# wanmeihuali/taichi_3d_gaussian_splatting

Hardware: NVIDIA H100
Metric: rendered Mpix/sec fwd+bwd @1080p, 1e6 Gaussians (higher is better)
Workload: dtype f32

## Files before the change

### taichi_3d_gaussian_splatting_b200/csrc/blend_bwd.cu

```cuda
#include "blend_bwd.cuh"

namespace gsb {

__device__ __forceinline__ void warp_transpose_reduce11(float (&v)[11], int lane) {
    {
        const bool hi = lane & 16;
#pragma unroll
        for (int i = 0; i < 5; ++i) {
            const float send = hi ? v[i] : v[i + 6];
            const float keep = hi ? v[i + 6] : v[i];
            v[i] = keep + __shfl_xor_sync(0xffffffffu, send, 16);
        }
        v[5] += __shfl_xor_sync(0xffffffffu, v[5], 16);
    }
    {
        const bool hi = lane & 8;
#pragma unroll
        for (int i = 0; i < 3; ++i) {
            const float send = hi ? v[i] : v[i + 3];
            const float keep = hi ? v[i + 3] : v[i];
            v[i] = keep + __shfl_xor_sync(0xffffffffu, send, 8);
        }
    }
    {
// ... 93 lines not shown
        if (block_start < warp_last) {
            const int skip = block_end - warp_last;
#pragma unroll 1
            for (int lw = skip > 0 ? (skip >> 5) : 0; lw < 8; ++lw) {
                unsigned int bits = s_bits[buf][warp][lw];
                if (skip > lw * 32) bits &= ~((1u << (skip - lw * 32)) - 1u);
                while (bits) {
                    const int j = lw * 32 + __ffs(bits) - 1;
                    bits &= bits - 1;
                    const int idx = block_end - 1 - j;
                    float v[11];
                    bool contributes;
                    {
                        const unsigned int ja = sb + j * 16;
                        const float4 r0 = lds128<0>(ja);
                        const float4 r1 = lds128<PLANE>(ja);
                        const float4 r2 = lds128<2 * PLANE>(ja);
                        const float d0 = px - r0.x, d1 = py - r0.y;
                        const float q0 = r0.z * d0 + r0.w * d1;
                        const float q1 = r0.w * d0 + r1.x * d1;
                        if (EXACT_EXP) {
                            const float gp = expf(-0.5f * (d0 * q0 + d1 * q1)) * r1.y;
                            const float opa = r1.z;
                            const float prod_alpha = gp * opa;
                            contributes = (idx < last) && (prod_alpha >= 1.0f / 255.0f);
                            const float alpha = fminf(prod_alpha, 0.99f);
                            const float inv = 1.0f / (1.0f - alpha);
                            const float Tn = T * inv;
                            const float aT = contributes ? alpha * Tn : 0.0f;
                            const float a_grad = contributes ? (r2.x * Tn - w0 * inv) * g0 + (r2.y * Tn - w1 * inv) * g1 +
                                                                   (r2.z * Tn - w2 * inv) * g2
                                                             : 0.0f;
                            T = contributes ? Tn : T;
                            w0 = fmaf(r2.x, aT, w0);
                            w1 = fmaf(r2.y, aT, w1);
                            w2 = fmaf(r2.z, aT, w2);
                            const float G = a_grad * opa * gp;
                            const float vs0 = G * q0, vs1 = G * q1;
                            if (STATS) {
                                mag0 += fabsf(vs0);
                                mag1 += fabsf(vs1);
                            }
                            v[0] = vs0;
                            v[1] = vs1;
                            v[2] = vs0 * q0;
                            v[3] = vs0 * q1;
                            v[4] = vs1 * q1;
                            v[5] = aT * g0;
                            v[6] = aT * g1;
                            v[7] = aT * g2;
                            v[8] = a_grad * gp * (1.0f - opa) * opa;
                            v[9] = STATS ? sqrtf(vs0 * vs0 + vs1 * vs1) : 0.0f;
                        } else {
                            const float P = fast_alpha(d0, d1, (-0.5f * GSB_L2E) * r0.z, -GSB_L2E * r0.w,
                                                       (-0.5f * GSB_L2E) * r1.x, r1.y);
                            contributes = (idx < last) && (P >= 1.0f / 255.0f);
                            const float alpha = fminf(P, 0.99f);
                            const float inv = rcp_approx(1.0f - alpha);
                            const float Tn = T * inv;
                            const float aT = contributes ? alpha * Tn : 0.0f;
                            const float cg = fmaf(r2.z, g2, fmaf(r2.y, g1, r2.x * g0));
                            const float a_grad = contributes ? fmaf(cg, Tn, -(w0 * inv)) : 0.0f;
                            T = contributes ? Tn : T;
                            w0 = fmaf(cg, aT, w0);
                            const float G = a_grad * P;
                            const float vs0 = G * q0, vs1 = G * q1;
                            if (STATS) {
                                mag0 += fabsf(vs0);
                                mag1 += fabsf(vs1);
                            }
                            v[0] = vs0;
                            v[1] = vs1;
                            v[2] = vs0 * q0;
                            v[3] = vs0 * q1;
                            v[4] = vs1 * q1;
                            v[5] = aT * g0;
                            v[6] = aT * g1;
                            v[7] = aT * g2;
                            v[8] = G * r1.z;
                            v[9] = STATS ? sqrt_approx(vs0 * vs0 + vs1 * vs1) : 0.0f;
                        }
                        v[10] = (STATS && contributes) ? 1.0f : 0.0f;
                    }
                    if (lane == 0) GSB_EMU_COUNT(EC_BF_VISITS, 1);
                    GSB_EMU_COUNT(EC_BF_PAIRS, contributes ? 1 : 0);
                    if (__any_sync(0xffffffffu, contributes)) {
                        if (lane == 0) GSB_EMU_COUNT(EC_BF_VISITS_ANY, 1);
                        warp_transpose_reduce11(v, lane);
                        if (red_writer && (STATS || red_slot < 9))
                            atomicAdd(p.accum + (size_t)s_off[buf][j] * GSB_ACCUM_FLOATS + red_slot, v[0]);
                    }
                }
            }
        }
    }
    if (STATS) {
        p.mag_image[2 * pix] = mag0;
        p.mag_image[2 * pix + 1] = mag1;
    }
}

#ifndef GSB_HOST_EMU
static BlendBwdParams make_blend_bwd_params(const GsbBackwardArgs &a, const Workspace &ws);

int launch_blend_backward_work(const GsbBackwardArgs &a, const Workspace &ws, unsigned long long *counters_dev,
                               cudaStream_t stream) {
    BlendBwdParams p = make_blend_bwd_params(a, ws);
    p.work_counters = counters_dev;
// ... 621 lines not shown
```

### taichi_3d_gaussian_splatting_b200/csrc/blend_bwd_transposed.cu

```cuda
#include <type_traits>

#include "blend_bwd.cuh"

namespace gsb {

#ifndef GSB_TB_CHUNK
#define GSB_TB_CHUNK 16
#endif
#ifndef GSB_TB_MIN_BLOCKS
#if GSB_TB_CHUNK == 8
#define GSB_TB_MIN_BLOCKS 4
#else
#define GSB_TB_MIN_BLOCKS 3
#endif
#endif
constexpr int TB_CHUNK = GSB_TB_CHUNK;
static_assert(TB_CHUNK == 8 || TB_CHUNK == 16, "a phase-2 lane takes whole rows of the 8 x 4 patch");
constexpr int TB_ROWS = TB_CHUNK / 8;
constexpr int TB_ROW = TB_CHUNK + 1;

struct TbWarp {
    float4 g[32];
    float4 chunk[3][TB_CHUNK];
    float2 x[32 * TB_ROW];
// ... 38 lines not shown

#ifndef GSB_TB_P1_UNROLL
#define GSB_TB_P1_UNROLL 4
#endif
constexpr int TB_P1_UNROLL = GSB_TB_P1_UNROLL;
static_assert(TB_CHUNK % TB_P1_UNROLL == 0, "a full chunk is a whole number of phase-1 groups");
__device__ __forceinline__ void red_add_f32x4(float *addr, const float4 v) {
#ifdef GSB_HOST_EMU
    atomicAdd(addr, v.x);
    atomicAdd(addr + 1, v.y);
    atomicAdd(addr + 2, v.z);
    atomicAdd(addr + 3, v.w);
#else
    atomicAdd(reinterpret_cast<float4 *>(addr), v);
#endif
}
__device__ __forceinline__ float keep_if_contributing(float P, int idx, int last) {
#ifdef GSB_HOST_EMU
    return ((idx < last) && (P >= 1.0f / 255.0f)) ? P : 0.0f;
#else
    float r;
    asm("{\n"
        ".reg .pred p, q;\n"
        "setp.lt.s32 q, %2, %3;\n"
        "setp.ge.and.f32 p, %1, 0f3B808081, q;\n"
        "selp.f32 %0, %1, 0f00000000, p;\n"
        "}\n"
        : "=f"(r)
        : "f"(P), "r"(idx), "r"(last));
    return r;
#endif
}

template <int CF>
using TbParams = typename std::conditional<CF == 0, BlendBwdParams, BlendBwdFeatParams>::type;

template <bool EXACT_EXP, bool STATS, bool COUNT = false, bool DEPTH = false, bool ALPHA = false, int CF = 0>
__global__ void __launch_bounds__(GSB_TILE_PIXELS, tb_min_blocks(CF))
blend_backward_transposed_kernel(const TbParams<CF> p) {
    static_assert(!(COUNT && (DEPTH || ALPHA || CF)), "the work-counter diagnostic runs the default arithmetic only");
    static_assert(CF % 4 == 0 && CF <= 16, "features: whole float4 groups");
    TbShared &S = *reinterpret_cast<TbShared *>(tb_dynamic_smem());
    constexpr int NV = STATS ? 11 : 9;
    constexpr int CFW = CF > 0 ? CF : 4;
    constexpr int P1U = CF >= 16 ? 2 : TB_P1_UNROLL;
    TbFeat<CFW> &SF = *reinterpret_cast<TbFeat<CFW> *>(tb_dynamic_smem() + sizeof(TbShared));

    const int tile = blockIdx.x;
    const int tu = tile % p.tiles_x, tv = tile / p.tiles_x;
    const int tid = threadIdx.x, lane = tid & 31, warp = tid >> 5;
    const int pu = tu * GSB_TILE_WIDTH + (warp & 1) * 8 + (lane & 7);
    const int pv = tv * GSB_TILE_HEIGHT + (warp >> 1) * 4 + (lane >> 3);
    const float px = (float)pu + 0.5f, py = (float)pv + 0.5f;
    const size_t pix = (size_t)pv * p.W + pu;
    const int start = p.tile_start[tile];

    const int last = p.last_effective[pix];
    float T = 1.0f - p.acc_alpha[pix];
    float w0 = 0.0f, w1 = 0.0f, w2 = 0.0f;
    const float g0 = p.grad_image[3 * pix], g1 = p.grad_image[3 * pix + 1], g2 = p.grad_image[3 * pix + 2];
    float mag0 = 0.0f, mag1 = 0.0f;
    unsigned int n_visits = 0, n_pairs = 0;
    float gd = 0.0f, hd = 0.0f, w3 = 0.0f;
    if (DEPTH) {
        const float Sa = p.acc_alpha[pix];
        gd = Sa > 0.0f ? p.grad_depth[pix] / Sa : 0.0f;
        hd = EXACT_EXP ? p.depth[pix] : gd * p.depth[pix];
    }
    float ga = 0.0f;
    if (ALPHA) {
        const float gs = p.grad_alpha[pix];
        ga = EXACT_EXP ? gs * T : DEPTH ? gs - hd : gs;
    }
    TbWarp &Wp = S.w[warp];
    Wp.g[lane] = make_float4(g0, g1, g2, gd);
    float gf[CFW];
    float wF;
    typename TbFeat<CFW>::Warp &WF = SF.w[warp];
    const BlendFeatureParams fp = feature_params(p);
    const int C = CF > 0 ? fp.channels : 0;
    if constexpr (CF > 0) {
        wF = 0.0f;
        const float *src = fp.grad_feature_map + pix * C;
#pragma unroll
        for (int c = 0; c < CF; ++c) gf[c] = c < C ? src[c] : 0.0f;
#pragma unroll
        for (int c = 0; c < CF; c += 4) WF.g[lane][c / 4] = make_float4(gf[c], gf[c + 1], gf[c + 2], gf[c + 3]);
    }

    const int ci = lane % TB_CHUNK, row0 = (lane / TB_CHUNK) * TB_ROWS;
    float2 *const x = Wp.x;
    float4 *const fin = reinterpret_cast<float4 *>(x);
    unsigned char *const list = Wp.list;

    int warp_last = last;
#pragma unroll
    for (int d = 16; d > 0; d >>= 1) warp_last = max(warp_last, __shfl_xor_sync(0xffffffffu, warp_last, d));
    if (tid == 0) {
        S.max_last = start;
        S.origin = make_float2((float)(tu * GSB_TILE_WIDTH), (float)(tv * GSB_TILE_HEIGHT));
    }
    __syncthreads();
    if (lane == 0) atomicMax(&S.max_last, warp_last);
    __syncthreads();
    const int end = min(p.tile_end[tile], S.max_last);

// ... 12 lines not shown
            {
                const int idx = block_end - 1 - tid;
                unsigned int mask = 0;
                if (idx >= block_start) {
                    const int o = __ldg(&p.sorted_vals[idx]);
                    const float4 *rec = p.records + 3 * (size_t)o;
                    const float4 r0 = __ldg(rec), r1 = __ldg(rec + 1);
                    if (EXACT_EXP) {
                        s_r0[tid] = r0;
                        s_r1[tid] = r1;
                    } else {
                        float4 f0, f1;
                        fast_planes(r0, r1, f0, f1);
                        s_r0[tid] = f0;
                        s_r1[tid] = f1;
                    }
                    float4 r2 = __ldg(rec + 2);
                    r2.w = __int_as_float(o);
                    s_r2[tid] = r2;
                    if constexpr (CF > 0) SF.row[buf][tid] = __ldg(&fp.point_id[o]);
                    mask = splat_patch_mask(r0.x, r0.y, r0.z, r0.w, r1.x, r1.y * r1.z, S.origin.x, S.origin.y);
                }
#pragma unroll
                for (int w = 0; w < 8; ++w) {
                    const unsigned int bits = __ballot_sync(0xffffffffu, (mask >> w) & 1u);
                    if (lane == 0) S.bits[buf][w][warp] = bits;
                }
            }
            __syncthreads();
            if (tid == 0) GSB_EMU_COUNT(EC_BATCHES, 1);
            if (block_start < warp_last) {
                const int skip = block_end - warp_last;
#pragma unroll
                for (int k = 0; k < 8; ++k) {
                    unsigned int bits = S.bits[buf][warp][k];
                    const int lo = skip - 32 * k;
                    if (lo >= 32) bits = 0u;
                    else if (lo > 0) bits &= ~((1u << lo) - 1u);
                    if ((bits >> lane) & 1u)
                        list[count + __popc(bits & ((1u << lane) - 1u))] = (unsigned char)(k * 32 + lane);
                    count += __popc(bits);
                }
                __syncwarp();
            }
        }

        int pos = 0;
#pragma unroll 1
        do {
            if (pos < count) {
                const int take = min(TB_CHUNK - have, count - pos);
                if (lane < take) {
                    const int j = list[pos + lane], slot = have + lane;
                    ck0[slot] = s_r0[j];
                    ck1[slot] = s_r1[j];
                    float4 r2 = s_r2[j];
                    ck_off[slot] = __float_as_int(r2.w);
                    r2.w = __int_as_float(block_end - 1 - j);
                    ck2[slot] = r2;
                    if constexpr (CF > 0) {
                        const int row = SF.row[buf][j];
                        WF.row[slot] = row;
                        const float *src = fp.features + (size_t)row * C;
#pragma unroll
                        for (int c = 0; c < CF; c += 4)
                            WF.f[slot][c / 4] = make_float4(c < C ? __ldg(src + c) : 0.0f, c + 1 < C ? __ldg(src + c + 1) : 0.0f,
                                                            c + 2 < C ? __ldg(src + c + 2) : 0.0f,
                                                            c + 3 < C ? __ldg(src + c + 3) : 0.0f);
                    }
                }
                have += take;
                pos += take;
                __syncwarp();
            }
            if (have == TB_CHUNK || (!real && have > 0)) {
                const int n = have;
                have = 0;
                if (COUNT) n_visits += (lane == 0) ? (unsigned int)n : 0u;
                if (lane == 0) {
                    GSB_EMU_COUNT(EC_TB_SPLATS, n);
                    GSB_EMU_COUNT(EC_TB_CHUNKS, 1);
                }
                const auto p1 = [&](const int i) -> float2 {
                    const float4 r0 = ck0[i];
                    const float4 r1 = ck1[i];
                    const float4 r2 = ck2[i];
                    const int idx = __float_as_int(r2.w);
                    const float d0 = px - r0.x, d1 = py - r0.y;
                    float sf = 0.0f;
                    if constexpr (CF > 0) {
#pragma unroll
                        for (int c = 0; c < CF; c += 4) {
                            const float4 f = WF.f[i][c / 4];
                            sf = fmaf(gf[c], f.x, sf);
                            sf = fmaf(gf[c + 1], f.y, sf);
                            sf = fmaf(gf[c + 2], f.z, sf);
                            sf = fmaf(gf[c + 3], f.w, sf);
                        }
                    }
                    float G, aT;
                    if (EXACT_EXP) {
                        const float q0 = r0.z * d0 + r0.w * d1;
                        const float q1 = r0.w * d0 + r1.x * d1;
                        const float gp = expf(-0.5f * (d0 * q0 + d1 * q1)) * r1.y;
                        const float prod_alpha = gp * r1.z;
                        const bool contributes = (idx < last) && (prod_alpha >= 1.0f / 255.0f);
                        const float alpha = fminf(prod_alpha, 0.99f);
                        const float inv = 1.0f / (1.0f - alpha);
                        const float Tn = T * inv;
                        aT = contributes ? alpha * Tn : 0.0f;
                        float a_grad = contributes ? (r2.x * Tn - w0 * inv) * g0 + (r2.y * Tn - w1 * inv) * g1 +
                                                         (r2.z * Tn - w2 * inv) * g2
                                                   : 0.0f;
                        if (DEPTH) {
                            const float e = r1.w - hd;
                            a_grad += contributes ? (e * Tn - w3 * inv) * gd : 0.0f;
                            w3 = fmaf(e, aT, w3);
                        }
                        if (ALPHA) a_grad += contributes ? ga * inv : 0.0f;
                        if constexpr (CF > 0) {
                            a_grad += contributes ? sf * Tn - wF * inv : 0.0f;
                            wF = fmaf(sf, aT, wF);
                        }
                        T = contributes ? Tn : T;
                        w0 = fmaf(r2.x, aT, w0);
                        w1 = fmaf(r2.y, aT, w1);
                        w2 = fmaf(r2.z, aT, w2);
                        G = a_grad * r1.z * gp;
                        if (STATS) {
                            mag0 += fabsf(G * q0);
                            mag1 += fabsf(G * q1);
                        }
                    } else {
                        float P = fast_alpha(d0, d1, r0.z, r0.w, r1.x, r1.y);
                        P = keep_if_contributing(P, idx, last);
                        const float alpha = fminf(P, 0.99f);
                        const float inv = rcp_approx(1.0f - alpha);
                        T *= inv;
                        aT = alpha * T;
                        float cg = fmaf(r2.z, g2, fmaf(r2.y, g1, ALPHA ? fmaf(r2.x, g0, ga) : r2.x * g0));
                        if (DEPTH) cg = ALPHA ? fmaf(gd, r1.w, cg) : fmaf(gd, r1.w, cg) - hd;
                        if constexpr (CF > 0) cg += sf;
                        const float a_grad = fmaf(cg, T, -(w0 * inv));
                        w0 = fmaf(cg, aT, w0);
                        G = a_grad * P;
                        if (STATS) {
                            const float q0 = (-2.0f / GSB_L2E) * fmaf(r0.z, d0, 0.5f * r0.w * d1);
                            const float q1 = (-2.0f / GSB_L2E) * fmaf(0.5f * r0.w, d0, r1.x * d1);
                            mag0 += fabsf(G * q0);
                            mag1 += fabsf(G * q1);
                        }
                    }
                    if (COUNT) n_pairs += aT > 0.0f ? 1u : 0u;
                    return make_float2(G, aT);
                };
                if (n == TB_CHUNK) {
#pragma unroll 1
                    for (int i0 = 0; i0 < TB_CHUNK; i0 += P1U) {
                        float2 ex[P1U];
#pragma unroll
                        for (int u = 0; u < P1U; ++u) ex[u] = p1(i0 + u);
#pragma unroll
                        for (int u = 0; u < P1U; ++u) x[lane * TB_ROW + i0 + u] = ex[u];
                    }
                } else {
#pragma unroll 1
                    for (int i = 0; i < n; ++i) x[lane * TB_ROW + i] = p1(i);
                }
                __syncwarp();

                const bool active = ci < n;
                float4 s0 = ck0[active ? ci : 0];
                float4 s1 = ck1[active ? ci : 0];
                if (!EXACT_EXP) {
                    s0.z *= -2.0f / GSB_L2E;
                    s0.w *= -1.0f / GSB_L2E;
                    s1.x *= -2.0f / GSB_L2E;
                }
                const float ca = s0.z, cb = s0.w, cc = s1.x;
                const float2 org = S.origin;
                const float pxc = org.x + (float)((warp & 1) * 8) + 4.0f;
                const float pyb = org.y + (float)((warp >> 1) * 4 + row0) + 0.5f;
                const float dxc = pxc - s0.x;
                float acc[12];
#pragma unroll
                for (int k = 0; k < 12; ++k) acc[k] = 0.0f;
                float af[CFW];
                if constexpr (CF > 0) {
#pragma unroll
                    for (int c = 0; c < CF; ++c) af[c] = 0.0f;
                }
                unsigned int nz = 0u;
#pragma unroll
                for (int row = 0; row < TB_ROWS; ++row) {
                    const float d1 = (pyb + (float)row) - s0.y;
                    const float q0r = fmaf(ca, dxc, cb * d1);
                    const float q1r = fmaf(cb, dxc, cc * d1);
                    float m0 = 0.0f, m1 = 0.0f, m2 = 0.0f;
#pragma unroll
                    for (int k = 0; k < 8; ++k) {
                        const float kc = (float)k - 3.5f;
                        const int pp = 8 * (row0 + row) + k;
                        const float2 ga = x[pp * TB_ROW + ci];
                        const float4 gp = Wp.g[pp];
                        m0 += ga.x;
                        m1 = fmaf(kc, ga.x, m1);
                        m2 = fmaf(kc * kc, ga.x, m2);
                        acc[5] = fmaf(ga.y, gp.x, acc[5]);
                        acc[6] = fmaf(ga.y, gp.y, acc[6]);
                        acc[7] = fmaf(ga.y, gp.z, acc[7]);
                        if (DEPTH) acc[11] = fmaf(ga.y, gp.w, acc[11]);
                        if (STATS) {
                            const float vs0 = ga.x * fmaf(ca, kc, q0r), vs1 = ga.x * fmaf(cb, kc, q1r);
                            const float mm = vs0 * vs0 + vs1 * vs1;
                            acc[9] += EXACT_EXP ? sqrtf(mm) : sqrt_approx(mm);
                            acc[10] += ga.y > 0.0f ? 1.0f : 0.0f;
                        }
                        nz |= __float_as_uint(ga.y);
                    }
                    const float t0 = fmaf(ca, m1, q0r * m0), t1 = fmaf(cb, m1, q1r * m0);
                    const float u0 = fmaf(ca, m2, q0r * m1), u1 = fmaf(cb, m2, q1r * m1);
                    acc[0] += t0;
                    acc[1] += t1;
                    acc[2] += fmaf(ca, u0, q0r * t0);
                    acc[3] += fmaf(cb, u0, q1r * t0);
                    acc[4] += fmaf(cb, u1, q1r * t1);
                    acc[8] += m0;
                }
                if constexpr (CF > 0) {
#pragma unroll 1
                    for (int row = 0; row < TB_ROWS; ++row) {
#pragma unroll 4
                        for (int k = 0; k < 8; ++k) {
                            const int pp = 8 * (row0 + row) + k;
                            const float aT = x[pp * TB_ROW + ci].y;
#pragma unroll
                            for (int c = 0; c < CF; c += 4) {
                                const float4 gc = WF.g[pp][c / 4];
                                af[c] = fmaf(aT, gc.x, af[c]);
                                af[c + 1] = fmaf(aT, gc.y, af[c + 1]);
                                af[c + 2] = fmaf(aT, gc.z, af[c + 2]);
                                af[c + 3] = fmaf(aT, gc.w, af[c + 3]);
                            }
                        }
                    }
                }
#pragma unroll
                for (int d = TB_CHUNK; d < 32; d *= 2) {
#pragma unroll
                    for (int k = 0; k < NV; ++k) acc[k] += __shfl_xor_sync(0xffffffffu, acc[k], d);
                    if (DEPTH) acc[11] += __shfl_xor_sync(0xffffffffu, acc[11], d);
                    if constexpr (CF > 0) {
#pragma unroll
                        for (int c = 0; c < CF; ++c) af[c] += __shfl_xor_sync(0xffffffffu, af[c], d);
                    }
                    nz |= __shfl_xor_sync(0xffffffffu, nz, d);
                }
                if constexpr (CF > 0) if (active && nz != 0u) {
                    constexpr int parts = 32 / TB_CHUNK;
                    const int h = lane / TB_CHUNK;
                    float *dst = fp.grad_features + (size_t)WF.row[ci] * C;
#pragma unroll
                    for (int c = 0; c < CF; c += 4) {
                        if ((c / 4) % parts != h || c >= C) continue;
                        if (C % 4 == 0) {
                            red_add_f32x4(dst + c, make_float4(af[c], af[c + 1], af[c + 2], af[c + 3]));
                        } else {
#pragma unroll
                            for (int k = 0; k < 4; ++k)
                                if (c + k < C) atomicAdd(dst + c + k, af[c + k]);
                        }
                    }
                }
                acc[8] *= EXACT_EXP ? (1.0f - s1.z) : s1.z;
                __syncwarp();
                if (lane < TB_CHUNK) {
                    if (!(active && nz != 0u)) ck_off[ci] = -1;
                    else GSB_EMU_COUNT(EC_TB_ROWS, 1);
                    fin[3 * ci] = make_float4(acc[0], acc[1], acc[2], acc[3]);
                    fin[3 * ci + 1] = make_float4(acc[4], acc[5], acc[6], acc[7]);
                    fin[3 * ci + 2] = make_float4(acc[8], STATS ? acc[9] : 0.0f, STATS ? acc[10] : 0.0f,
                                                  DEPTH ? acc[11] : 0.0f);
                }
                __syncwarp();
#pragma unroll
                for (int e0 = 0; e0 < 3 * TB_CHUNK; e0 += 32) {
                    const int e = e0 + lane, row = e / 3;
                    if (e < 3 * TB_CHUNK) {
                        const int o = ck_off[row];
                        if (o >= 0) red_add_f32x4(p.accum + (size_t)o * GSB_ACCUM_FLOATS + 4 * (e - 3 * row), fin[e]);
                    }
                }
                __syncwarp();
            }
        } while (pos < count);
        if (!real) break;
    }
    if (STATS) {
        p.mag_image[2 * pix] = mag0;
        p.mag_image[2 * pix + 1] = mag1;
    }
    if (COUNT) {
#pragma unroll
        for (int d = 16; d > 0; d >>= 1) {
            n_visits += __shfl_xor_sync(0xffffffffu, n_visits, d);
            n_pairs += __shfl_xor_sync(0xffffffffu, n_pairs, d);
        }
        if (lane == 0) {
            atomicAdd(p.work_counters, (unsigned long long)n_visits);
            atomicAdd(p.work_counters + 1, (unsigned long long)n_pairs);
        }
    }
}

#ifndef GSB_HOST_EMU
template <bool EXACT_EXP, bool STATS, bool DEPTH = false, bool ALPHA = false, int CF = 0>
static int launch_tb(const TbParams<CF> &p, int tiles, cudaStream_t stream) {
    static bool configured = false;
    if (!configured) {
        GSB_CUDA_CHECK(cudaFuncSetAttribute(blend_backward_transposed_kernel<EXACT_EXP, STATS, false, DEPTH, ALPHA, CF>,
                                            cudaFuncAttributeMaxDynamicSharedMemorySize, (int)tb_smem_bytes<CF>()));
        configured = true;
    }
    blend_backward_transposed_kernel<EXACT_EXP, STATS, false, DEPTH, ALPHA, CF>
        <<<tiles, GSB_TILE_PIXELS, tb_smem_bytes<CF>(), stream>>>(p);
    GSB_CUDA_CHECK(cudaGetLastError());
    return GSB_OK;
}

template <bool DEPTH, bool ALPHA, int CF = 0>
static int launch_tb_terms(const TbParams<CF> &p, int tiles, bool exact_exp, bool stats, cudaStream_t stream) {
    if (exact_exp)
        return stats ? launch_tb<true, true, DEPTH, ALPHA, CF>(p, tiles, stream)
                     : launch_tb<true, false, DEPTH, ALPHA, CF>(p, tiles, stream);
    return stats ? launch_tb<false, true, DEPTH, ALPHA, CF>(p, tiles, stream)
                 : launch_tb<false, false, DEPTH, ALPHA, CF>(p, tiles, stream);
}

template <int CF>
static int launch_tb_features(const BlendBwdFeatParams &p, int tiles, bool exact_exp, bool stats, cudaStream_t stream, bool depth,
                              bool alpha) {
    if (alpha)
        return depth ? launch_tb_terms<true, true, CF>(p, tiles, exact_exp, stats, stream)
                     : launch_tb_terms<false, true, CF>(p, tiles, exact_exp, stats, stream);
    return depth ? launch_tb_terms<true, false, CF>(p, tiles, exact_exp, stats, stream)
                 : launch_tb_terms<false, false, CF>(p, tiles, exact_exp, stats, stream);
}

int launch_blend_backward_transposed(const BlendBwdParams &p, int tiles, bool exact_exp, bool stats,
                                     cudaStream_t stream, bool depth, bool alpha, const BlendFeatureParams *feat) {
    if (feat) {
        BlendBwdFeatParams fp;
        static_cast<BlendBwdParams &>(fp) = p;
// ... 24 lines not shown
```

### taichi_3d_gaussian_splatting_b200/csrc/blend_fwd.cu

```cuda
#include <type_traits>

#include "common.cuh"

namespace gsb {

struct BlendFwdParams {
    int H, W, tiles_x;
    const int *tile_start;
    const int *tile_end;
    const int *sorted_vals;
    const float4 *records;
    float *image;
    float *depth;
    float *acc_alpha;
    int *last_effective;
    int *valid_count;
    unsigned long long *work_counters;
};
struct BlendFwdFeatParams : BlendFwdParams {
    int channels;
    const int *point_id;
    const float *features;
    float *out_features;
};
template <int CF>
using FwParams = typename std::conditional<CF == 0, BlendFwdParams, BlendFwdFeatParams>::type;
struct FwFeatureArgs {
    int channels;
    const int *point_id;
    const float *features;
    float *out_features;
};
__device__ __forceinline__ FwFeatureArgs feature_args(const BlendFwdParams &) { return FwFeatureArgs{0, nullptr, nullptr, nullptr}; }
__device__ __forceinline__ FwFeatureArgs feature_args(const BlendFwdFeatParams &p) {
    return FwFeatureArgs{p.channels, p.point_id, p.features, p.out_features};
}

#ifdef GSB_HOST_EMU
static inline float *fw_feature_smem() { return reinterpret_cast<float *>(simt_emu::dynamic_smem()); }
#else
extern __shared__ __align__(16) float gsb_fw_dynamic_smem[];
__device__ __forceinline__ float *fw_feature_smem() { return gsb_fw_dynamic_smem; }
#endif

__device__ __forceinline__ float ex2_approx(float x) { return ex2_mufu(x); }

__device__ __forceinline__ void count_if_blended(float wgt, int idx, int &cnt, int &last) {
#ifdef GSB_HOST_EMU
    if (wgt > 0.0f) {
        cnt += 1;
        last = idx;
    }
#else
    asm("{\n"
        ".reg .pred p;\n"
        "setp.gt.f32 p, %2, 0f00000000;\n"
        "@p add.s32 %0, %0, 1;\n"
        "@p mov.b32 %1, %3;\n"
        "}\n"
        : "+r"(cnt), "+r"(last)
        : "f"(wgt), "r"(idx));
#endif
}

#ifndef GSB_FWD_MIN_BLOCKS
#define GSB_FWD_MIN_BLOCKS 4
#endif
#ifndef GSB_FWD_UNROLL
#define GSB_FWD_UNROLL 8
#endif
constexpr int FW_UNROLL = GSB_FWD_UNROLL;
constexpr int FW_CHUNK = 32;
template <int CF>
__device__ __forceinline__ const float4 *fw_feature_row(int buf, int j) {
    return reinterpret_cast<const float4 *>(fw_feature_smem() + (buf * GSB_TILE_PIXELS + j) * CF);
}
constexpr int fw_min_blocks(int cf, bool exact_exp) { return cf == 0 ? GSB_FWD_MIN_BLOCKS : (cf <= 8 && !exact_exp) ? 3 : 2; }
constexpr int fw_feature_smem_bytes(int cf) { return 2 * GSB_TILE_PIXELS * cf * (int)sizeof(float); }

template <bool RGB_ONLY, bool EXACT_EXP, bool COUNT = false, int CF = 0>
__global__ void __launch_bounds__(GSB_TILE_PIXELS, fw_min_blocks(CF, EXACT_EXP))
blend_forward_kernel(const FwParams<CF> p) {
    static_assert(CF == 0 || (CF % 4 == 0 && !RGB_ONLY && !COUNT), "features: whole float4 groups, full outputs only");
    __shared__ float4 s_rec[2 * 3 * GSB_TILE_PIXELS];
    __shared__ unsigned int s_bits[2][8][8];
    __shared__ float4 s_chunk[8][3][FW_CHUNK];
    __shared__ unsigned char s_list[8][GSB_TILE_PIXELS];

    const int tile = blockIdx.x;
    const int tu = tile % p.tiles_x, tv = tile / p.tiles_x;
    const int tid = threadIdx.x, lane = tid & 31, warp = tid >> 5;
    const int pu = tu * GSB_TILE_WIDTH + (warp & 1) * 8 + (lane & 7);
    const int pv = tv * GSB_TILE_HEIGHT + (warp >> 1) * 4 + (lane >> 3);
    const float px = (float)pu + 0.5f, py = (float)pv + 0.5f;
    const float tile_x0 = (float)(tu * GSB_TILE_WIDTH), tile_y0 = (float)(tv * GSB_TILE_HEIGHT);
    const int start = p.tile_start[tile], end = p.tile_end[tile];

    float T = 1.0f, Tlive = 1.0f, C0 = 0.0f, C1 = 0.0f, C2 = 0.0f, D = 0.0f, Wt = 0.0f;
    int last = start, cnt = 0;
    unsigned int n_visits = 0, n_pairs = 0;
    unsigned int n_p84 = 0, n_p88 = 0, n_p164 = 0, n_p44 = 0;
    float4 *const ck0 = s_chunk[warp][0], *const ck1 = s_chunk[warp][1], *const ck2 = s_chunk[warp][2];
    unsigned char *const list = s_list[warp];
    const unsigned int lt_mask = (1u << lane) - 1u;
    constexpr int CFW = CF > 0 ? CF : 4;
    const FwFeatureArgs fa = feature_args(p);
    float F[CFW];
#pragma unroll
    for (int c = 0; c < CFW; ++c) F[c] = 0.0f;

    int buf = 0;
    for (int base = start; base < end; base += GSB_TILE_PIXELS, buf ^= 1) {
        float4 *const s_r0 = s_rec + buf * 3 * GSB_TILE_PIXELS;
        float4 *const s_r1 = s_r0 + GSB_TILE_PIXELS, *const s_r2 = s_r0 + 2 * GSB_TILE_PIXELS;
        const int idx = base + tid;
        unsigned int mask = 0;
        if (idx < end) {
            const int o = __ldg(&p.sorted_vals[idx]);
            const float4 *rec = p.records + 3 * (size_t)o;
            const float4 r0 = __ldg(rec), r1 = __ldg(rec + 1);
            if (EXACT_EXP) {
                s_r0[tid] = r0;
                s_r1[tid] = r1;
            } else {
                float4 f0, f1;
                fast_planes(r0, r1, f0, f1);
                s_r0[tid] = f0;
                s_r1[tid] = f1;
            }
            s_r2[tid] = __ldg(rec + 2);
            if constexpr (CF > 0) {
                const int C = fa.channels;
                const float *src = fa.features + (size_t)__ldg(&fa.point_id[o]) * C;
                float4 *dst = reinterpret_cast<float4 *>(fw_feature_smem() + (buf * GSB_TILE_PIXELS + tid) * CF);
#pragma unroll
                for (int c = 0; c < CF; c += 4)
                    dst[c / 4] = make_float4(c < C ? __ldg(src + c) : 0.0f, c + 1 < C ? __ldg(src + c + 1) : 0.0f,
                                             c + 2 < C ? __ldg(src + c + 2) : 0.0f, c + 3 < C ? __ldg(src + c + 3) : 0.0f);
            }
            mask = splat_patch_mask(r0.x, r0.y, r0.z, r0.w, r1.x, r1.y * r1.z, tile_x0, tile_y0);
            if (COUNT) {
                n_p84 += __popc(mask);
                n_p88 += __popc((mask | (mask >> 2)) & 0x33u);
                n_p164 += __popc((mask | (mask >> 1)) & 0x55u);
                const SplatReach rr = make_splat_reach(r0.z, r0.w, r1.x, r1.y * r1.z);
                if (rr.mode == 2) n_p44 += 16;
                else if (rr.mode == 1)
                    for (int q = 0; q < 16; ++q) {
                        const float X0 = tile_x0 + 4.0f * (q & 3) + 0.5f - r0.x, Y0 = tile_y0 + 4.0f * (q >> 2) + 0.5f - r0.y;
                        n_p44 += rect_reachable(rr, X0, X0 + 3.0f, Y0, Y0 + 3.0f) ? 1 : 0;
                    }
            }
        }
#pragma unroll
        for (int w = 0; w < 8; ++w) {
            const unsigned int bits = __ballot_sync(0xffffffffu, (mask >> w) & 1u);
            if (lane == 0) s_bits[buf][w][warp] = bits;
        }
        if (__syncthreads_and(!(T > 0.0f))) break;
        if (__all_sync(0xffffffffu, !(T > 0.0f))) continue;
        int count = 0;
#pragma unroll
        for (int k = 0; k < 8; ++k) {
            const unsigned int bits = s_bits[buf][warp][k];
            if ((bits >> lane) & 1u) list[count + __popc(bits & lt_mask)] = (unsigned char)(k * 32 + lane);
            count += __popc(bits);
        }
        __syncwarp();
#pragma unroll 1
        for (int pos = 0; pos < count; pos += FW_CHUNK) {
            const int n = min(FW_CHUNK, count - pos);
            if (lane < n) {
                const int j = list[pos + lane];
                ck0[lane] = s_r0[j];
                ck1[lane] = s_r1[j];
                float4 r2 = s_r2[j];
                r2.w = __int_as_float(base + j + 1);
                ck2[lane] = r2;
            }
            __syncwarp();
            if (COUNT) n_visits += (lane == 0) ? (unsigned int)n : 0u;
            if (lane == 0) GSB_EMU_COUNT(EC_FW_VISITS, n);
#pragma unroll FW_UNROLL
            for (int i = 0; i < n; ++i) {
                const float4 r0 = ck0[i];
                const float4 r1 = ck1[i];
                const float4 r2 = ck2[i];
                const float dx = px - r0.x, dy = py - r0.y;
                if (EXACT_EXP) {
                    const float power = -0.5f * (dx * dx * r0.z + dy * dy * r1.x) - dx * dy * r0.w;
                    float alpha = expf(power) * r1.y * r1.z;
                    if (!(alpha < 1.0f / 255.0f)) {
                        if (COUNT) n_pairs += T > 0.0f ? 1u : 0u;
                        GSB_EMU_COUNT(EC_FW_PAIRS, 1);
                        alpha = fminf(alpha, 0.99f);
                        const float nT = T * (1.0f - alpha);
                        if (nT >= 0.0001f) {
                            last = __float_as_int(r2.w);
                            C0 += r2.x * alpha * T;
                            C1 += r2.y * alpha * T;
                            C2 += r2.z * alpha * T;
                            if (!RGB_ONLY) {
                                D += r1.w * alpha * T;
                                Wt += alpha * T;
                                cnt += 1;
                            }
                            if constexpr (CF > 0) {
                                const float4 *fi = fw_feature_row<CF>(buf, __float_as_int(r2.w) - 1 - base);
#pragma unroll
                                for (int c = 0; c < CF; c += 4) {
                                    const float4 f = fi[c / 4];
                                    F[c] += f.x * alpha * T;
                                    F[c + 1] += f.y * alpha * T;
                                    F[c + 2] += f.z * alpha * T;
                                    F[c + 3] += f.w * alpha * T;
                                }
                            }
                            T = nT;
                            Tlive = nT;
                        } else {
                            T = 0.0f;
                        }
                    }
                } else {
                    float P = fast_alpha(dx, dy, r0.z, r0.w, r1.x, r1.y);
                    P = (P < 1.0f / 255.0f) ? 0.0f : P;
                    const float alpha = fminf(P, 0.99f);
                    const float nT = T * (1.0f - alpha);
                    const bool ok = nT >= 0.0001f;
                    const float wgt = ok ? alpha * T : 0.0f;
                    if (COUNT) n_pairs += (P != 0.0f && T > 0.0f) ? 1u : 0u;
                    GSB_EMU_COUNT(EC_FW_PAIRS, (P != 0.0f && T > 0.0f) ? 1 : 0);
                    C0 = fmaf(r2.x, wgt, C0);
                    C1 = fmaf(r2.y, wgt, C1);
                    C2 = fmaf(r2.z, wgt, C2);
                    if (!RGB_ONLY) {
                        D = fmaf(r1.w, wgt, D);
                        Wt += wgt;
                        count_if_blended(wgt, __float_as_int(r2.w), cnt, last);
                    }
                    if constexpr (CF > 0) {
                        const float4 *fi = fw_feature_row<CF>(buf, __float_as_int(r2.w) - 1 - base);
#pragma unroll
                        for (int c = 0; c < CF; c += 4) {
                            const float4 f = fi[c / 4];
                            F[c] = fmaf(f.x, wgt, F[c]);
                            F[c + 1] = fmaf(f.y, wgt, F[c + 1]);
                            F[c + 2] = fmaf(f.z, wgt, F[c + 2]);
                            F[c + 3] = fmaf(f.w, wgt, F[c + 3]);
                        }
                    }
                    T = ok ? nT : -fabsf(T);
                }
            }
            __syncwarp();
            if (__all_sync(0xffffffffu, !(T > 0.0f))) break;
        }
    }
    const size_t pix = (size_t)pv * p.W + pu;
    p.image[3 * pix] = C0;
    p.image[3 * pix + 1] = C1;
    p.image[3 * pix + 2] = C2;
    if (!RGB_ONLY) {
        p.depth[pix] = D / fmaxf(Wt, 1e-6f);
        p.acc_alpha[pix] = 1.0f - (EXACT_EXP ? Tlive : fabsf(T));
        p.last_effective[pix] = last;
        p.valid_count[pix] = cnt;
    }
    if constexpr (CF > 0) {
        const int C = fa.channels;
#pragma unroll
        for (int c = 0; c < CF; ++c)
            if (c < C) fa.out_features[pix * C + c] = F[c];
    }
    if (COUNT) {
#pragma unroll
        for (int d = 16; d > 0; d >>= 1) {
            n_visits += __shfl_xor_sync(0xffffffffu, n_visits, d);
            n_pairs += __shfl_xor_sync(0xffffffffu, n_pairs, d);
            n_p84 += __shfl_xor_sync(0xffffffffu, n_p84, d);
            n_p88 += __shfl_xor_sync(0xffffffffu, n_p88, d);
            n_p164 += __shfl_xor_sync(0xffffffffu, n_p164, d);
            n_p44 += __shfl_xor_sync(0xffffffffu, n_p44, d);
        }
        if (lane == 0) {
            atomicAdd(p.work_counters, (unsigned long long)n_visits);
            atomicAdd(p.work_counters + 1, (unsigned long long)n_pairs);
            atomicAdd(p.work_counters + 2, (unsigned long long)n_p84);
            atomicAdd(p.work_counters + 3, (unsigned long long)n_p88);
            atomicAdd(p.work_counters + 4, (unsigned long long)n_p164);
            atomicAdd(p.work_counters + 5, (unsigned long long)n_p44);
        }
    }
}

#ifndef GSB_HOST_EMU
template <bool EXACT_EXP, int CF>
static int launch_fwd_features(const BlendFwdFeatParams &p, int tiles, cudaStream_t stream) {
    static bool configured = false;
    if (!configured) {
        GSB_CUDA_CHECK(cudaFuncSetAttribute(blend_forward_kernel<false, EXACT_EXP, false, CF>,
                                            cudaFuncAttributeMaxDynamicSharedMemorySize, fw_feature_smem_bytes(CF)));
        configured = true;
    }
    blend_forward_kernel<false, EXACT_EXP, false, CF><<<tiles, GSB_TILE_PIXELS, fw_feature_smem_bytes(CF), stream>>>(p);
// ... 76 lines not shown
```

### taichi_3d_gaussian_splatting_b200/csrc/common.cuh

```cuda
#pragma once
#include <cuda_runtime.h>
#include <stdint.h>

#include "../../include/gsb200.h"

#define GSB_TILE_PIXELS (GSB_TILE_WIDTH * GSB_TILE_HEIGHT)

namespace gsb {

void set_error(const char *fmt, ...);
#define GSB_CUDA_CHECK(expr)                                                                   \
    do {                                                                                       \
        cudaError_t _e = (expr);                                                               \
        if (_e != cudaSuccess) {                                                               \
            gsb::set_error("%s failed: %s (%s:%d)", #expr, cudaGetErrorString(_e), __FILE__,   \
                           __LINE__);                                                          \
            return GSB_ECUDA;                                                                  \
        }                                                                                      \
    } while (0)

enum Counter { CNT_M = 0, CNT_K = 1, CNT_OVERFLOW = 2, CNT_MAX_DEPTH_KEY = 4 };
enum Ticket { TICKET_SCAN = 0, TICKET_SORT0 = 1  };

struct PoseBlock {
// ... 113 lines not shown
    float y;
    asm("rcp.approx.ftz.f32 %0, %1;" : "=f"(y) : "f"(x));
    return y;
}
#endif
__device__ __forceinline__ float quad_form(const SplatReach &r, float dx, float dy) {
    return fmaf(dx, fmaf(r.b2, dy, r.a * dx), r.c * dy * dy);
}
__device__ __forceinline__ SplatReach make_splat_reach(float a, float b, float c, float rescale_times_opacity) {
    SplatReach r;
    r.a = a; r.b2 = 2.0f * b; r.c = c;
    const float ro = rescale_times_opacity;
    r.nb_ic = -b * rcp_fast(c);
    r.nb_ia = -b * rcp_fast(a);
    r.t2 = fmaf(2.0f * 1.002f, __logf(fmaxf(255.0f * ro, 1.0f)), 1e-3f);
    const float det = a * c - b * b;
    if (!(ro == ro) || !(det > 0.0f) || !(a > 0.0f) || !(c > 0.0f)) r.mode = 2;
    else if (ro < (1.0f / 255.0f) * 0.999f) r.mode = 0;
    else r.mode = 1;
    return r;
}
__device__ __forceinline__ bool rect_reachable(const SplatReach &r, float X0, float X1, float Y0, float Y1) {
    if (X0 <= 0.0f && X1 >= 0.0f && Y0 <= 0.0f && Y1 >= 0.0f) return true;
    const float ya = fminf(fmaxf(r.nb_ic * X0, Y0), Y1);
    const float yb = fminf(fmaxf(r.nb_ic * X1, Y0), Y1);
    const float xa = fminf(fmaxf(r.nb_ia * Y0, X0), X1);
    const float xb = fminf(fmaxf(r.nb_ia * Y1, X0), X1);
    const float best = fminf(fminf(quad_form(r, X0, ya), quad_form(r, X1, yb)),
                             fminf(quad_form(r, xa, Y0), quad_form(r, xb, Y1)));
    return !(best > r.t2);
}

__device__ __forceinline__ unsigned int splat_patch_mask(float u, float v, float a, float b, float c,
                                                         float rescale_times_opacity, float tile_x0,
                                                         float tile_y0) {
    const SplatReach r = make_splat_reach(a, b, c, rescale_times_opacity);
    if (r.mode == 0) return 0u;
    if (r.mode == 2) return 0xFFu;
    unsigned int m = 0;
#pragma unroll
    for (int w = 0; w < 8; ++w) {
        const float X0 = tile_x0 + 8.0f * (w & 1) + 0.5f - u;
        const float Y0 = tile_y0 + 4.0f * (w >> 1) + 0.5f - v;
        if (rect_reachable(r, X0, X0 + 7.0f, Y0, Y0 + 3.0f)) m |= 1u << w;
    }
    return m;
}
#endif

#if defined(__CUDACC__) || defined(GSB_HOST_EMU)
constexpr float GSB_L2E = 1.4426950408889634f;
#ifdef GSB_HOST_EMU
__device__ __forceinline__ float ex2_mufu(float x) { return exp2f(x); }
#else
__device__ __forceinline__ float ex2_mufu(float x) {
    float y;
    asm("ex2.approx.ftz.f32 %0, %1;" : "=f"(y) : "f"(x));
    return y;
}
#endif
__device__ __forceinline__ float fast_alpha(float dx, float dy, float A, float B, float C, float ro) {
    return ex2_mufu(fmaf(dx, fmaf(A, dx, B * dy), (C * dy) * dy)) * ro;
}
__device__ __forceinline__ void fast_planes(const float4 r0, const float4 r1, float4 &s0, float4 &s1) {
    s0 = make_float4(r0.x, r0.y, (-0.5f * GSB_L2E) * r0.z, -GSB_L2E * r0.w);
    s1 = make_float4((-0.5f * GSB_L2E) * r1.x, r1.y * r1.z, 1.0f - r1.z, r1.w);
}
#endif

#if defined(__CUDACC__) || defined(GSB_HOST_EMU)
#ifdef GSB_HOST_EMU
__device__ __forceinline__ void mbar_init(unsigned long long *bar, unsigned int) { *bar = 0; }
__device__ __forceinline__ void mbar_arrive_expect_tx(unsigned long long *, unsigned int) {}
__device__ __forceinline__ void bulk_copy_g2s(void *dst_smem, const void *src_gmem, unsigned int bytes,
                                              unsigned long long *) {
    memcpy(dst_smem, src_gmem, bytes);
}
__device__ __forceinline__ void mbar_wait(unsigned long long *, unsigned int) { simt_emu::warp_exchange(0u); }
__device__ __forceinline__ void fence_proxy_async_smem() {}
#else
__device__ __forceinline__ unsigned int smem_addr(const void *p) {
    return (unsigned int)__cvta_generic_to_shared(p);
}
__device__ __forceinline__ void mbar_init(unsigned long long *bar, unsigned int count) {
    asm volatile("mbarrier.init.shared::cta.b64 [%0], %1;" ::"r"(smem_addr(bar)), "r"(count));
    asm volatile("fence.mbarrier_init.release.cluster;" ::: "memory");
}
__device__ __forceinline__ void mbar_arrive_expect_tx(unsigned long long *bar, unsigned int bytes) {
    asm volatile("mbarrier.arrive.expect_tx.shared::cta.b64 _, [%0], %1;" ::"r"(smem_addr(bar)),
                 "r"(bytes)
                 : "memory");
}
__device__ __forceinline__ void bulk_copy_g2s(void *dst_smem, const void *src_gmem, unsigned int bytes,
                                              unsigned long long *bar) {
    asm volatile(
        "cp.async.bulk.shared::cluster.global.mbarrier::complete_tx::bytes [%0], [%1], %2, [%3];" ::"r"(
            smem_addr(dst_smem)),
        "l"(src_gmem), "r"(bytes), "r"(smem_addr(bar))
        : "memory");
}
__device__ __forceinline__ void mbar_wait(unsigned long long *bar, unsigned int parity) {
    asm volatile(
        "{\n"
        ".reg .pred p;\n"
        "WAIT_LOOP:\n"
        "mbarrier.try_wait.parity.shared::cta.b64 p, [%0], %1;\n"
        "@p bra WAIT_DONE;\n"
        "bra WAIT_LOOP;\n"
        "WAIT_DONE:\n"
        "}\n" ::"r"(smem_addr(bar)),
        "r"(parity)
        : "memory");
}
__device__ __forceinline__ void fence_proxy_async_smem() { asm volatile("fence.proxy.async.shared::cta;" ::: "memory"); }
#endif

#endif

#ifdef GSB_HOST_EMU
// ... 29 lines not shown
```

Before: 1299.

## Re-expand Gaussian exponent per warp patch centre and fold opacity into log2 term

```diff
diff --git a/taichi_3d_gaussian_splatting_b200/csrc/blend_bwd.cu b/taichi_3d_gaussian_splatting_b200/csrc/blend_bwd.cu
--- a/taichi_3d_gaussian_splatting_b200/csrc/blend_bwd.cu
+++ b/taichi_3d_gaussian_splatting_b200/csrc/blend_bwd.cu
@@ -169,8 +169,11 @@
                             v[8] = a_grad * gp * (1.0f - opa) * opa;
                             v[9] = STATS ? sqrtf(vs0 * vs0 + vs1 * vs1) : 0.0f;
                         } else {
-                            const float P = fast_alpha(d0, d1, (-0.5f * GSB_L2E) * r0.z, -GSB_L2E * r0.w,
-                                                       (-0.5f * GSB_L2E) * r1.x, r1.y);
+                            float4 c0, c1;
+                            patch_planes(make_float4(r0.x, r0.y, (-0.5f * GSB_L2E) * r0.z, -GSB_L2E * r0.w),
+                                         make_float4((-0.5f * GSB_L2E) * r1.x, r1.y, r1.z, r1.w), patch_cx(tile_x0, warp),
+                                         patch_cy(tile_y0, warp), c0, c1);
+                            const float P = patch_alpha(c0, c1, patch_lane(lane));
                             contributes = (idx < last) && (P >= 1.0f / 255.0f);
                             const float alpha = fminf(P, 0.99f);
                             const float inv = rcp_approx(1.0f - alpha);
diff --git a/taichi_3d_gaussian_splatting_b200/csrc/blend_bwd_transposed.cu b/taichi_3d_gaussian_splatting_b200/csrc/blend_bwd_transposed.cu
--- a/taichi_3d_gaussian_splatting_b200/csrc/blend_bwd_transposed.cu
+++ b/taichi_3d_gaussian_splatting_b200/csrc/blend_bwd_transposed.cu
@@ -114,6 +114,7 @@
     const int pu = tu * GSB_TILE_WIDTH + (warp & 1) * 8 + (lane & 7);
     const int pv = tv * GSB_TILE_HEIGHT + (warp >> 1) * 4 + (lane >> 3);
     const float px = (float)pu + 0.5f, py = (float)pv + 0.5f;
+    const PatchLane L = patch_lane(lane);
     const size_t pix = (size_t)pv * p.W + pu;
     const int start = p.tile_start[tile];
 
@@ -232,8 +233,16 @@
                 const int take = min(TB_CHUNK - have, count - pos);
                 if (lane < take) {
                     const int j = list[pos + lane], slot = have + lane;
-                    ck0[slot] = s_r0[j];
-                    ck1[slot] = s_r1[j];
+                    if (EXACT_EXP) {
+                        ck0[slot] = s_r0[j];
+                        ck1[slot] = s_r1[j];
+                    } else {
+                        float4 c0, c1;
+                        const float2 org = S.origin;
+                        patch_planes(s_r0[j], s_r1[j], patch_cx(org.x, warp), patch_cy(org.y, warp), c0, c1);
+                        ck0[slot] = c0;
+                        ck1[slot] = c1;
+                    }
                     float4 r2 = s_r2[j];
                     ck_off[slot] = __float_as_int(r2.w);
                     r2.w = __int_as_float(block_end - 1 - j);
@@ -266,7 +275,6 @@
                     const float4 r1 = ck1[i];
                     const float4 r2 = ck2[i];
                     const int idx = __float_as_int(r2.w);
-                    const float d0 = px - r0.x, d1 = py - r0.y;
                     float sf = 0.0f;
                     if constexpr (CF > 0) {
 #pragma unroll
@@ -280,6 +288,7 @@
                     }
                     float G, aT;
                     if (EXACT_EXP) {
+                        const float d0 = px - r0.x, d1 = py - r0.y;
                         const float q0 = r0.z * d0 + r0.w * d1;
                         const float q1 = r0.w * d0 + r1.x * d1;
                         const float gp = expf(-0.5f * (d0 * q0 + d1 * q1)) * r1.y;
@@ -312,7 +321,7 @@
                             mag1 += fabsf(G * q1);
                         }
                     } else {
-                        float P = fast_alpha(d0, d1, r0.z, r0.w, r1.x, r1.y);
+                        float P = patch_alpha(r0, r1, L);
                         P = keep_if_contributing(P, idx, last);
                         const float alpha = fminf(P, 0.99f);
                         const float inv = rcp_approx(1.0f - alpha);
@@ -325,8 +334,8 @@
                         w0 = fmaf(cg, aT, w0);
                         G = a_grad * P;
                         if (STATS) {
-                            const float q0 = (-2.0f / GSB_L2E) * fmaf(r0.z, d0, 0.5f * r0.w * d1);
-                            const float q1 = (-2.0f / GSB_L2E) * fmaf(0.5f * r0.w, d0, r1.x * d1);
+                            const float q0 = (-1.0f / GSB_L2E) * fmaf(2.0f * r0.w, L.i, fmaf(r1.x, L.j, r0.y));
+                            const float q1 = (-1.0f / GSB_L2E) * fmaf(r1.x, L.i, fmaf(2.0f * r1.y, L.j, r0.z));
                             mag0 += fabsf(G * q0);
                             mag1 += fabsf(G * q1);
                         }
@@ -350,18 +359,23 @@
                 __syncwarp();
 
                 const bool active = ci < n;
-                float4 s0 = ck0[active ? ci : 0];
-                float4 s1 = ck1[active ? ci : 0];
-                if (!EXACT_EXP) {
-                    s0.z *= -2.0f / GSB_L2E;
-                    s0.w *= -1.0f / GSB_L2E;
-                    s1.x *= -2.0f / GSB_L2E;
-                }
-                const float ca = s0.z, cb = s0.w, cc = s1.x;
-                const float2 org = S.origin;
-                const float pxc = org.x + (float)((warp & 1) * 8) + 4.0f;
-                const float pyb = org.y + (float)((warp >> 1) * 4 + row0) + 0.5f;
-                const float dxc = pxc - s0.x;
+                const float4 s0 = ck0[active ? ci : 0];
+                const float4 s1 = ck1[active ? ci : 0];
+                float ca, cb, cc, dxc = 0.0f, pyb = 0.0f, q0c = 0.0f, q1c = 0.0f;
+                if (EXACT_EXP) {
+                    const float2 org = S.origin;
+                    ca = s0.z;
+                    cb = s0.w;
+                    cc = s1.x;
+                    dxc = (org.x + (float)((warp & 1) * 8) + 4.0f) - s0.x;
+                    pyb = org.y + (float)((warp >> 1) * 4 + row0) + 0.5f;
+                } else {
+                    ca = (-2.0f / GSB_L2E) * s0.w;
+                    cb = (-1.0f / GSB_L2E) * s1.x;
+                    cc = (-2.0f / GSB_L2E) * s1.y;
+                    q0c = (-1.0f / GSB_L2E) * s0.y;
+                    q1c = (-1.0f / GSB_L2E) * s0.z;
+                }
                 float acc[12];
 #pragma unroll
                 for (int k = 0; k < 12; ++k) acc[k] = 0.0f;
@@ -373,9 +387,16 @@
                 unsigned int nz = 0u;
 #pragma unroll
                 for (int row = 0; row < TB_ROWS; ++row) {
-                    const float d1 = (pyb + (float)row) - s0.y;
-                    const float q0r = fmaf(ca, dxc, cb * d1);
-                    const float q1r = fmaf(cb, dxc, cc * d1);
+                    float q0r, q1r;
+                    if (EXACT_EXP) {
+                        const float d1 = (pyb + (float)row) - s0.y;
+                        q0r = fmaf(ca, dxc, cb * d1);
+                        q1r = fmaf(cb, dxc, cc * d1);
+                    } else {
+                        const float jr = (float)(row0 + row) - 1.5f;
+                        q0r = fmaf(cb, jr, q0c);
+                        q1r = fmaf(cc, jr, q1c);
+                    }
                     float m0 = 0.0f, m1 = 0.0f, m2 = 0.0f;
 #pragma unroll
                     for (int k = 0; k < 8; ++k) {
@@ -477,8 +498,11 @@
         if (!real) break;
     }
     if (STATS) {
-        p.mag_image[2 * pix] = mag0;
-        p.mag_image[2 * pix + 1] = mag1;
+        const int t = opaque_int(tile);
+        const size_t q = (size_t)((t / p.tiles_x) * GSB_TILE_HEIGHT + (warp >> 1) * 4 + (lane >> 3)) * p.W +
+                         (t % p.tiles_x) * GSB_TILE_WIDTH + (warp & 1) * 8 + (lane & 7);
+        p.mag_image[2 * q] = mag0;
+        p.mag_image[2 * q + 1] = mag1;
     }
     if (COUNT) {
 #pragma unroll
diff --git a/taichi_3d_gaussian_splatting_b200/csrc/blend_fwd.cu b/taichi_3d_gaussian_splatting_b200/csrc/blend_fwd.cu
--- a/taichi_3d_gaussian_splatting_b200/csrc/blend_fwd.cu
+++ b/taichi_3d_gaussian_splatting_b200/csrc/blend_fwd.cu
@@ -45,21 +45,54 @@
 
 __device__ __forceinline__ float ex2_approx(float x) { return ex2_mufu(x); }
 
-__device__ __forceinline__ void count_if_blended(float wgt, int idx, int &cnt, int &last) {
+template <bool COUNTS>
+__device__ __forceinline__ float blend_step(float P, float &T, int idx, int &cnt, int &last) {
+    const float alpha = fminf(P, 0.99f);
+    const float aT = alpha * T;
+    const float nT = fmaf(-alpha, T, T);
 #ifdef GSB_HOST_EMU
-    if (wgt > 0.0f) {
-        cnt += 1;
-        last = idx;
-    }
+    float wgt = 0.0f;
+    if (!(P < 1.0f / 255.0f)) {
+        if (nT >= 0.0001f) {
+            wgt = aT;
+            T = nT;
+            if (COUNTS) {
+                cnt += 1;
+                last = idx;
+            }
+        } else {
+            T = -fabsf(T);
+        }
+    }
+    return wgt;
 #else
-    asm("{\n"
-        ".reg .pred p;\n"
-        "setp.gt.f32 p, %2, 0f00000000;\n"
-        "@p add.s32 %0, %0, 1;\n"
-        "@p mov.b32 %1, %3;\n"
-        "}\n"
-        : "+r"(cnt), "+r"(last)
-        : "f"(wgt), "r"(idx));
+    float wgt;
+    if (COUNTS) {
+        asm("{\n"
+            ".reg .pred pc, pb, pn;\n"
+            "setp.geu.f32 pc, %4, 0f3B808081;\n"
+            "setp.ge.and.f32 pb|pn, %5, 0f38D1B717, pc;\n"
+            "selp.f32 %0, %6, 0f00000000, pb;\n"
+            "@pb mov.f32 %1, %5;\n"
+            "@pn or.b32 %1, %1, 0x80000000;\n"
+            "@pb add.s32 %2, %2, 1;\n"
+            "@pb mov.b32 %3, %7;\n"
+            "}\n"
+            : "=f"(wgt), "+f"(T), "+r"(cnt), "+r"(last)
+            : "f"(P), "f"(nT), "f"(aT), "r"(idx));
+    } else {
+        asm("{\n"
+            ".reg .pred pc, pb, pn;\n"
+            "setp.geu.f32 pc, %2, 0f3B808081;\n"
+            "setp.ge.and.f32 pb|pn, %3, 0f38D1B717, pc;\n"
+            "selp.f32 %0, %4, 0f00000000, pb;\n"
+            "@pb mov.f32 %1, %3;\n"
+            "@pn or.b32 %1, %1, 0x80000000;\n"
+            "}\n"
+            : "=f"(wgt), "+f"(T)
+            : "f"(P), "f"(nT), "f"(aT));
+    }
+    return wgt;
 #endif
 }
 
@@ -138,7 +171,7 @@
                     dst[c / 4] = make_float4(c < C ? __ldg(src + c) : 0.0f, c + 1 < C ? __ldg(src + c + 1) : 0.0f,
                                              c + 2 < C ? __ldg(src + c + 2) : 0.0f, c + 3 < C ? __ldg(src + c + 3) : 0.0f);
             }
-            mask = splat_patch_mask(r0.x, r0.y, r0.z, r0.w, r1.x, r1.y * r1.z, tile_x0, tile_y0);
+            mask = splat_patch_mask(r0.x, r0.y, r0.z, r0.w, r1.x, r1.y * r1.z, opaque_float(tile_x0), opaque_float(tile_y0));
             if (COUNT) {
                 n_p84 += __popc(mask);
                 n_p88 += __popc((mask | (mask >> 2)) & 0x33u);
@@ -167,13 +200,22 @@
             count += __popc(bits);
         }
         __syncwarp();
+        const PatchLane L = patch_lane(opaque_int(lane));
 #pragma unroll 1
         for (int pos = 0; pos < count; pos += FW_CHUNK) {
             const int n = min(FW_CHUNK, count - pos);
             if (lane < n) {
                 const int j = list[pos + lane];
-                ck0[lane] = s_r0[j];
-                ck1[lane] = s_r1[j];
+                if (EXACT_EXP) {
+                    ck0[lane] = s_r0[j];
+                    ck1[lane] = s_r1[j];
+                } else {
+                    float4 c0, c1;
+                    patch_planes(s_r0[j], s_r1[j], patch_cx(opaque_float(tile_x0), warp), patch_cy(opaque_float(tile_y0), warp),
+                                 c0, c1);
+                    ck0[lane] = c0;
+                    ck1[lane] = c1;
+                }
                 float4 r2 = s_r2[j];
                 r2.w = __int_as_float(base + j + 1);
                 ck2[lane] = r2;
@@ -186,8 +228,8 @@
                 const float4 r0 = ck0[i];
                 const float4 r1 = ck1[i];
                 const float4 r2 = ck2[i];
-                const float dx = px - r0.x, dy = py - r0.y;
                 if (EXACT_EXP) {
+                    const float dx = px - r0.x, dy = py - r0.y;
                     const float power = -0.5f * (dx * dx * r0.z + dy * dy * r1.x) - dx * dy * r0.w;
                     float alpha = expf(power) * r1.y * r1.z;
                     if (!(alpha < 1.0f / 255.0f)) {
@@ -223,21 +265,16 @@
                         }
                     }
                 } else {
-                    float P = fast_alpha(dx, dy, r0.z, r0.w, r1.x, r1.y);
-                    P = (P < 1.0f / 255.0f) ? 0.0f : P;
-                    const float alpha = fminf(P, 0.99f);
-                    const float nT = T * (1.0f - alpha);
-                    const bool ok = nT >= 0.0001f;
-                    const float wgt = ok ? alpha * T : 0.0f;
-                    if (COUNT) n_pairs += (P != 0.0f && T > 0.0f) ? 1u : 0u;
-                    GSB_EMU_COUNT(EC_FW_PAIRS, (P != 0.0f && T > 0.0f) ? 1 : 0);
+                    const float P = patch_alpha(r0, r1, L);
+                    if (COUNT) n_pairs += (!(P < 1.0f / 255.0f) && T > 0.0f) ? 1u : 0u;
+                    GSB_EMU_COUNT(EC_FW_PAIRS, (!(P < 1.0f / 255.0f) && T > 0.0f) ? 1 : 0);
+                    const float wgt = blend_step<!RGB_ONLY>(P, T, __float_as_int(r2.w), cnt, last);
                     C0 = fmaf(r2.x, wgt, C0);
                     C1 = fmaf(r2.y, wgt, C1);
                     C2 = fmaf(r2.z, wgt, C2);
                     if (!RGB_ONLY) {
                         D = fmaf(r1.w, wgt, D);
                         Wt += wgt;
-                        count_if_blended(wgt, __float_as_int(r2.w), cnt, last);
                     }
                     if constexpr (CF > 0) {
                         const float4 *fi = fw_feature_row<CF>(buf, __float_as_int(r2.w) - 1 - base);
@@ -250,7 +287,6 @@
                             F[c + 3] = fmaf(f.w, wgt, F[c + 3]);
                         }
                     }
-                    T = ok ? nT : -fabsf(T);
                 }
             }
             __syncwarp();
diff --git a/taichi_3d_gaussian_splatting_b200/csrc/common.cuh b/taichi_3d_gaussian_splatting_b200/csrc/common.cuh
--- a/taichi_3d_gaussian_splatting_b200/csrc/common.cuh
+++ b/taichi_3d_gaussian_splatting_b200/csrc/common.cuh
@@ -189,19 +189,60 @@
 constexpr float GSB_L2E = 1.4426950408889634f;
 #ifdef GSB_HOST_EMU
 __device__ __forceinline__ float ex2_mufu(float x) { return exp2f(x); }
+__device__ __forceinline__ float lg2_mufu(float x) { return log2f(x); }
 #else
 __device__ __forceinline__ float ex2_mufu(float x) {
     float y;
     asm("ex2.approx.ftz.f32 %0, %1;" : "=f"(y) : "f"(x));
     return y;
 }
-#endif
-__device__ __forceinline__ float fast_alpha(float dx, float dy, float A, float B, float C, float ro) {
-    return ex2_mufu(fmaf(dx, fmaf(A, dx, B * dy), (C * dy) * dy)) * ro;
-}
+__device__ __forceinline__ float lg2_mufu(float x) {
+    float y;
+    asm("lg2.approx.ftz.f32 %0, %1;" : "=f"(y) : "f"(x));
+    return y;
+}
+#endif
 __device__ __forceinline__ void fast_planes(const float4 r0, const float4 r1, float4 &s0, float4 &s1) {
     s0 = make_float4(r0.x, r0.y, (-0.5f * GSB_L2E) * r0.z, -GSB_L2E * r0.w);
     s1 = make_float4((-0.5f * GSB_L2E) * r1.x, r1.y * r1.z, 1.0f - r1.z, r1.w);
+}
+__device__ __forceinline__ void patch_planes(const float4 s0, const float4 s1, float cx, float cy, float4 &c0, float4 &c1) {
+    const float A = s0.z, B = s0.w, C = s1.x;
+    const float Dx = cx - s0.x, Dy = cy - s0.y;
+    const float a1 = fmaf(2.0f * A, Dx, B * Dy);
+    const float a2 = fmaf(B, Dx, (2.0f * C) * Dy);
+    const float a0 = fmaf(Dx, fmaf(A, Dx, B * Dy), fmaf(C * Dy, Dy, lg2_mufu(s1.y)));
+    c0 = make_float4(a0, a1, a2, A);
+    c1 = make_float4(B, C, s1.z, s1.w);
+}
+__device__ __forceinline__ int opaque_int(int x) {
+#ifndef GSB_HOST_EMU
+    asm volatile("" : "+r"(x));
+#endif
+    return x;
+}
+__device__ __forceinline__ float opaque_float(float x) {
+#ifndef GSB_HOST_EMU
+    asm volatile("" : "+f"(x));
+#endif
+    return x;
+}
+struct PatchLane {
+    float i, j, ii, ij, jj;
+};
+__device__ __forceinline__ PatchLane patch_lane(int lane) {
+    PatchLane L;
+    L.i = (float)(lane & 7) - 3.5f;
+    L.j = (float)(lane >> 3) - 1.5f;
+    L.ii = L.i * L.i;
+    L.ij = L.i * L.j;
+    L.jj = L.j * L.j;
+    return L;
+}
+__device__ __forceinline__ float patch_cx(float tile_x0, int warp) { return tile_x0 + (float)((warp & 1) * 8 + 4); }
+__device__ __forceinline__ float patch_cy(float tile_y0, int warp) { return tile_y0 + (float)((warp >> 1) * 4 + 2); }
+__device__ __forceinline__ float patch_alpha(const float4 c0, const float4 c1, const PatchLane &L) {
+    return ex2_mufu(fmaf(c1.y, L.jj, fmaf(c1.x, L.ij, fmaf(c0.w, L.ii, fmaf(c0.z, L.j, fmaf(c0.y, L.i, c0.x))))));
 }
 #endif
 
```

New measurement: 1313, median of 6. 1.01x the previous value.
